# jzhou316/meta-gcn

Measured on AMD Instinct MI355X. Metric: edges/sec GCN fwd+bwd, 10M-edge synth graph F=128, at 1/2/4/8 MI355X, higher is better.
Workload: dtype f32; 1 GPU; config2: Erdos-Renyi N=1M, E=10M (+1M self-loops), F=128, 3-layer GCN (sm, add, bias, ReLU) fwd+bwd; nodes=1000000, edges=10000000, nnz=11000000, feat=128, layers=3, global_batch=1, parallelism=single

## Files before the change

meta-gcn_amd/csrc/fused.hip:

```cpp

#include <string>

#include "mgcn_internal.h"
#include "x6.h"

#ifndef MGCN_NT_AUX
#define MGCN_NT_AUX 2
#endif
#ifndef MGCN_NT_OUT
#define MGCN_NT_OUT 2
#endif

namespace mgcn {
namespace {

using namespace x6;

constexpr int kXwF = 128;
constexpr int kXwRows = 32;
constexpr int kXwWaves = 8;
constexpr int kXwThreads = 64 * kXwWaves;
constexpr int kXwImg = kXwRows * 256;
constexpr int kXwStageLd = kXwF + 8;
constexpr int kXwStage = kXwRows * kXwStageLd * 4;
// ... 1496 lines not shown
  }
  if (EPI != EPI_STORE || HCS) {
    __syncthreads();
    if constexpr (EPI != EPI_STORE) {
      if (tid < kXwF) {
        const float *red = reinterpret_cast<const float *>(lds);
        float s = 0.0f;
#pragma unroll
        for (int l = 0; l < 16; ++l) s = __fadd_rn(s, red[l * kXwF + tid]);
        a.colsum_partial[(int64_t)blockIdx.x * kXwF + tid] = s;
      }
    }
    if (HCS && tid >= kXwF && tid < 2 * kXwF) {
      const int f = tid - kXwF;
      const float *red2 = reinterpret_cast<const float *>(lds) + 16 * kXwF;
      float s = 0.0f;
#pragma unroll
      for (int l = 0; l < 16; ++l) s = __fadd_rn(s, red2[l * kXwF + f]);
      A.hcs_partial[(int64_t)blockIdx.x * kXwF + f] = s;
    }
  }
  XTAIL_EXIT(1, n_my);
}

int g_xw_ws_full = 1;
int g_xw_ws_max = 1;

int bs_grid() {
  int dev = 0, cus = 256;
  if (hipGetDevice(&dev) != hipSuccess ||
      hipDeviceGetAttribute(&cus, hipDeviceAttributeMultiprocessorCount, dev) != hipSuccess)
    cus = 256;
  return cus;
}

template <int U, int MODE, int ROLL>
int launch_bs_ur(const XbsArgs &a, int epi, int grid, hipStream_t s) {
  if (epi == EPI_RELU_DIV)
    hipLaunchKernelGGL((spmm_xw_bwd_ws_kernel<U, EPI_RELU_DIV, MODE, ROLL>), dim3(grid),
                       dim3(kBsThreads), 0, s, a);
  else if (epi == EPI_RELU)
    hipLaunchKernelGGL((spmm_xw_bwd_ws_kernel<U, EPI_RELU, MODE, ROLL>), dim3(grid),
                       dim3(kBsThreads), 0, s, a);
  else
    hipLaunchKernelGGL((spmm_xw_bwd_ws_kernel<U, EPI_STORE, MODE, ROLL>), dim3(grid),
                       dim3(kBsThreads), 0, s, a);
  return check_launch("spmm_xw_bwd_ws_kernel");
}

int g_bs_roll = 2;

template <int U, int MODE>
int launch_bs_u(const XbsArgs &a, int epi, int grid, hipStream_t s) {
  if constexpr (MODE == kBsDwsM) {
    return launch_bs_ur<U, MODE, 0>(a, epi, grid, s);
  } else {
    return g_bs_roll == 0 ? launch_bs_ur<U, MODE, 0>(a, epi, grid, s)
                          : launch_bs_ur<U, MODE, 2>(a, epi, grid, s);
  }
}

int g_bs_dbg = 0;

int g_bs_full_unroll = 5;

template <int MODE>
int launch_bs(const XbsArgs &a, int epi, int grid, hipStream_t s) {
  if constexpr (MODE == kBsDwsM) {
    return launch_bs_u<3, MODE>(a, epi, grid, s);
  } else {
    return g_bs_full_unroll == 4 ? launch_bs_u<4, MODE>(a, epi, grid, s)
         : g_bs_full_unroll == 5 ? launch_bs_u<5, MODE>(a, epi, grid, s)
                                 : launch_bs_u<6, MODE>(a, epi, grid, s);
  }
}

int bs_prepare(XbsArgs &sa) {
  sa.dbg = MGCN_EXPERIMENT ? g_bs_dbg : 0;
  sa.spin = g_spin_limit;
  sa.err = device_error_word();
  return sa.err == nullptr ? MGCN_EHIP : MGCN_OK;
}

}

int xw_set_ws(const char *name, int value) {
  const std::string n(name);
  auto flag = [&](int &g) {
    if (value < 0 || value > 1) {
      set_error("%s must be 0 or 1", name);
      return (int)MGCN_EINVAL;
    }
    g = value;
    return (int)MGCN_OK;
  };
  auto unroll = [&](int &g, std::initializer_list<int> ok) {
    for (int v : ok)
      if (v == value) {
        g = value;
        return (int)MGCN_OK;
      }
    set_error("%s: unsupported value %d", name, value);
    return (int)MGCN_EINVAL;
  };
  if (n == "xw_pk_unroll" || n == "xw_pk_bwd_unroll") {
    if (!MGCN_EXPERIMENT) {
      set_error("%s: experiment builds only (make exp -> libmgcn_exp.so)", name);
      return MGCN_EINVAL;
    }
    return n == "xw_pk_unroll" ? unroll(g_xw_pk_unroll, {3, 4, 5, 6})
                               : unroll(g_xw_pk_bwd_unroll, {2, 3, 4});
  }
  if (n == "xw_ws_max") return flag(g_xw_ws_max);
  if (n == "xw_ws_roll") return unroll(g_bs_roll, {0, 2});
  if (n == "xw_ws_full") return flag(g_xw_ws_full);
  if (n == "xw_ws_dbg") {
    if (!MGCN_EXPERIMENT) {
      set_error("xw_ws_dbg: experiment builds only (make exp -> libmgcn_exp.so)");
      return MGCN_EINVAL;
    }
    g_bs_dbg = value;
    return MGCN_OK;
  }
  return unroll(g_bs_full_unroll, {4, 5, 6});
}

int xw_set_dyn_rounds(int value) {
  if (value < 0 || value > 64) {
    set_error("xw_dyn_rounds must be in 0 .. 64 (0: no dynamic claim)");
    return MGCN_EINVAL;
  }
  g_xw_dyn_rounds = value;
  return MGCN_OK;
}

int xw_set_unroll(int value) {
  if (value != 4 && value != 5 && value != 6 && value != 8) {
    set_error("spmm_xw_unroll must be 4, 5, 6 or 8 (5 / 6: the forward only)");
    return MGCN_EINVAL;
  }
  g_xw_unroll = value;
  return MGCN_OK;
}

}

using namespace mgcn;

extern "C" int mgcn_spmm_xw_supported(int32_t F_in, int32_t F_out, int reduce) {
  return F_in == F_out && (F_in == kXwF || F_in == 256) && gemm_precision_is_x6() &&
         (reduce == MGCN_REDUCE_SUM || reduce == MGCN_REDUCE_MEAN);
}

extern "C" int mgcn_spmm_xw_bwd_full_supported(int32_t F_in, int32_t F_out) {
  return F_in == kXwF && F_out == kXwF && gemm_precision_is_x6();
}

extern "C" size_t mgcn_spmm_xw_fwd_workspace_bytes(int32_t F_in, int32_t F_out) {
  if (F_in == kXwF && F_out == kXwF) return xw_dyn_workspace_bytes();
  return F_in == 256 && F_out == 256 ? xw_wide_workspace_bytes(false) : 0;
}

namespace {
inline bool aligned16(const void *p) { return reinterpret_cast<uintptr_t>(p) % 16 == 0; }

int check_fwd_outputs(const char *who, bool wide, int32_t F_in, const float *bias,
                      const uint32_t *relu_mask, const float *Z, int64_t ldz) {
  MGCN_REQUIRE(wide || bias == nullptr || reinterpret_cast<uintptr_t>(bias) % 4 == 0,
               "%s: bias not 4-byte aligned", who);
  MGCN_REQUIRE(relu_mask == nullptr || aligned16(relu_mask), "%s: relu_mask not 16-byte aligned",
               who);
  MGCN_REQUIRE(Z == nullptr || (ldz >= F_in && ldz % 4 == 0 && aligned16(Z) &&
                                (wide || (uint64_t)kXwRows * (uint64_t)ldz * 4u < (1ull << 31))),
               "%s: Z must have 16-byte aligned rows (ldz >= F_in)", who);
  return MGCN_OK;
}

XwArgs xw_args(int64_t n_rows, const int64_t *rowptr, const int32_t *col, const float *w,
               const float *W, int64_t ldw, const float *bias, float *Y, int64_t ldy, int reduce,
               int relu, uint32_t *relu_mask, float *Z, int64_t ldz) {
  XwArgs a{};
  a.n_rows = n_rows;
  a.rowptr = rowptr;
  a.col = col;
  a.w = w;
  a.W = W;
  a.ldw = ldw;
  a.bias = bias;
  a.Y = Y;
  a.ldy = ldy;
  a.relu_mask = relu_mask;
  a.Z = Z;
  a.ldz = ldz;
  a.mean = reduce == MGCN_REDUCE_MEAN;
  a.relu = relu != 0;
// ... 7 lines not shown
int check_bwd_outputs(const char *who, bool wide, int64_t n_rows, int32_t F_in, int32_t F_out,
                      const float *W, int64_t ldw, const float *dX, int64_t lddx,
                      const uint32_t *relu_mask, const void *workspace, size_t workspace_bytes) {
  if (wide)
    MGCN_REQUIRE(W != nullptr && ldw >= F_out && lddx >= F_in && lddx % 4 == 0 && aligned16(dX) &&
                     (uint64_t)16 * (uint64_t)lddx * 4u < (1ull << 31),
                 "%s: bad W/dX (16-byte aligned dX rows)", who);
  else
    MGCN_REQUIRE(W == nullptr || (ldw % 4 == 0 && aligned16(W)),
                 "%s: W must have 16-byte aligned rows", who);
  MGCN_REQUIRE(relu_mask == nullptr || aligned16(relu_mask), "%s: relu_mask not 16-byte aligned",
               who);
  return require_workspace(who, workspace, workspace_bytes,
                           mgcn_spmm_xw_bwd_workspace_bytes(n_rows, F_in, F_out));
}

XbArgs xb_args(int64_t n_rows, const int64_t *rowptr_t, const int32_t *col_t, const float *w_t,
               const float *row_scale, const float *W, int64_t ldw, float *dX, int64_t lddx,
               const uint32_t *relu_mask, const float *row_div, void *workspace) {
  XbArgs a{};
  a.n_rows = n_rows;
  a.rowptr = rowptr_t;
  a.col = col_t;
  a.w = w_t;
  a.row_scale = row_scale;
  a.W = W;
  a.ldw = ldw;
  a.dX = dX;
  a.lddx = lddx;
  a.relu_mask = relu_mask;
  a.row_div = row_div;
  a.dw_partial = static_cast<float *>(workspace);
  a.colsum_partial = reinterpret_cast<float *>(static_cast<char *>(workspace) +
                                               align_up((size_t)xw_grid() * kXwF * kXwF * 4, 256));
  return a;
}
}

extern "C" int mgcn_spmm_xw_fwd(int64_t n_rows, int64_t n_cols, int32_t F_in, int32_t F_out,
                                const int64_t *rowptr, const int32_t *col, const float *w,
                                const float *X, int64_t ldx, const float *W, int64_t ldw,
                                const float *bias, float *Y, int64_t ldy, int reduce, int relu,
                                uint32_t *relu_mask, float *Z, int64_t ldz, void *workspace,
                                size_t workspace_bytes, void *stream) {
  clear_error();
  if (int rc = take_device_error()) return rc;
  MGCN_REQUIRE(n_rows >= 0, "mgcn_spmm_xw_fwd: negative size");
  MGCN_REQUIRE(mgcn_spmm_xw_supported(F_in, F_out, reduce),
               "mgcn_spmm_xw_fwd: unsupported F_in=%d F_out=%d reduce=%d (needs 128 x 128 or "
               "256 x 256, sum/mean, bf16x6)",
               F_in, F_out, reduce);
  MGCN_REQUIRE(relu_mask == nullptr || relu, "mgcn_spmm_xw_fwd: relu_mask needs relu");
  if (n_rows == 0) return MGCN_OK;
  MGCN_REQUIRE(rowptr && X && W && Y, "mgcn_spmm_xw_fwd: null array");
  MGCN_REQUIRE(ldx >= F_in && ldx % 4 == 0 && reinterpret_cast<uintptr_t>(X) % 16 == 0,
               "mgcn_spmm_xw_fwd: X must have 16-byte aligned rows");
  MGCN_REQUIRE(ldw >= F_out && ldy >= F_out, "mgcn_spmm_xw_fwd: leading dimension too small");
  if (F_in == 256) {
    MGCN_REQUIRE(n_cols > 0 && (uint64_t)16 * (uint64_t)(ldy > ldz ? ldy : ldz) * 4u < (1ull << 31),
                 "mgcn_spmm_xw_fwd: leading dimension too large");
    if (int rc = check_fwd_outputs("mgcn_spmm_xw_fwd", true, F_in, bias, relu_mask, Z, ldz))
      return rc;
    MGCN_REQUIRE(ldy % 4 == 0 && aligned16(Y),
                 "mgcn_spmm_xw_fwd: Y must have 16-byte aligned rows at F = 256");
    if (int rc = require_workspace("mgcn_spmm_xw_fwd", workspace, workspace_bytes,
                                   mgcn_spmm_xw_fwd_workspace_bytes(F_in, F_out)))
      return rc;
    return xw_wide_fwd(n_rows, rowptr, col, w, X, ldx, W, ldw, bias, Y, ldy,
                       reduce == MGCN_REDUCE_MEAN, relu != 0, relu_mask, Z, ldz, workspace,
                       as_stream(stream));
  }
  MGCN_REQUIRE(n_cols > 0 && (uint64_t)n_cols * (uint64_t)ldx * 4u <= 0xfffffff0ull,
               "mgcn_spmm_xw_fwd: X must hold 1 .. 4 GiB - 1 bytes (32-bit gather offsets)");
  MGCN_REQUIRE((uint64_t)kXwRows * (uint64_t)ldy * 4u < (1ull << 31),
               "mgcn_spmm_xw_fwd: ldy too large");
  if (int rc = check_fwd_outputs("mgcn_spmm_xw_fwd", false, F_in, bias, relu_mask, Z, ldz))
    return rc;
  XwArgs a = xw_args(n_rows, rowptr, col, w, W, ldw, bias, Y, ldy, reduce, relu, relu_mask, Z, ldz);
  a.X = X;
  a.ldx = ldx;
  a.n_cols = n_cols;
  hipStream_t s = as_stream(stream);
  int rc = MGCN_OK;
  if (launch_xw_dyn(a, workspace, workspace_bytes, s, &rc)) return rc;
  return g_xw_unroll == 4 ? launch_xw<4>(a, s)
       : g_xw_unroll == 5 ? launch_xw<5>(a, s)
       : g_xw_unroll == 6 ? launch_xw<6>(a, s)
                          : launch_xw<8>(a, s);
}

extern "C" size_t mgcn_spmm_xw_bwd_workspace_bytes(int64_t n_rows, int32_t F_in, int32_t F_out) {
  (void)n_rows;
  if (F_in == 256 && F_out == 256) return xw_wide_workspace_bytes(true);
  const size_t g = (size_t)xw_grid();
  return align_up(g * kXwF * kXwF * 4, 256) + align_up(g * kXwF * 4, 256);
}

namespace {
int xw_bwd_impl(int64_t n_rows, int64_t n_cols, int32_t F_in, int32_t F_out,
                const int64_t *rowptr_t, const int32_t *col_t, const float *w_t,
                const float *row_scale, const float *dY, int64_t lddy, const float *X,
                int64_t ldx, const float *W, int64_t ldw, float *dW, int64_t lddw, int accumulate,
                float *dX, int64_t lddx, const uint32_t *relu_mask, const float *row_div,
                float *colsum, const uint32_t *win_mask, const int32_t *slot_map,
                float *dy_colsum, void *workspace, size_t workspace_bytes, void *stream) {
  if (int rc = take_device_error()) return rc;
  MGCN_REQUIRE(n_rows >= 0, "mgcn_spmm_xw_bwd: negative size");
  MGCN_REQUIRE((win_mask == nullptr) == (slot_map == nullptr),
               "mgcn_spmm_xw_bwd: win_mask and slot_map go together (max adjoint)");
  MGCN_REQUIRE(mgcn_spmm_xw_supported(F_in, F_out, MGCN_REDUCE_SUM),
               "mgcn_spmm_xw_bwd: unsupported F_in=%d F_out=%d (needs 128 x 128 or 256 x 256, "
               "bf16x6)", F_in, F_out);
  const bool dx_only = X == nullptr && dW == nullptr;
  MGCN_REQUIRE(dx_only || mgcn_spmm_xw_bwd_full_supported(F_in, F_out),
               "mgcn_spmm_xw_bwd: at F=%d only the dX-only form (X = dW = NULL)", F_in);
  MGCN_REQUIRE(dx_only || (X != nullptr && dW != nullptr && lddw >= F_out),
               "mgcn_spmm_xw_bwd: bad dW (X and dW are given together, or both NULL for dX only)");
  MGCN_REQUIRE(row_div == nullptr || relu_mask != nullptr,
               "mgcn_spmm_xw_bwd: row_div needs relu_mask");
  hipStream_t s = as_stream(stream);
  if (n_rows == 0) {
    if (dy_colsum) MGCN_HIP_TRY(hipMemsetAsync(dy_colsum, 0, sizeof(float) * F_out, s));
    if (!accumulate && dW != nullptr)
      for (int32_t r = 0; r < F_in; ++r)
        MGCN_HIP_TRY(hipMemsetAsync(dW + r * lddw, 0, sizeof(float) * F_out, s));
    if (colsum && !(dx_only && accumulate))
      MGCN_HIP_TRY(hipMemsetAsync(colsum, 0, sizeof(float) * F_in, s));
    return MGCN_OK;
  }
  MGCN_REQUIRE(!dx_only || (dX != nullptr && win_mask == nullptr),
               "mgcn_spmm_xw_bwd: the dX-only form needs dX and takes no win_mask");
  const int epi = epi_of(relu_mask, row_div);
  MGCN_REQUIRE(epi == EPI_STORE || (dX != nullptr && colsum != nullptr),
               "mgcn_spmm_xw_bwd: relu_mask needs dX and colsum");
  MGCN_REQUIRE(rowptr_t && dY, "mgcn_spmm_xw_bwd: null array");
  MGCN_REQUIRE(lddy >= F_out && lddy % 4 == 0 && reinterpret_cast<uintptr_t>(dY) % 16 == 0,
               "mgcn_spmm_xw_bwd: dY must have 16-byte aligned rows");
  if (F_in == 256) {
    MGCN_REQUIRE(dX != nullptr && win_mask == nullptr, "mgcn_spmm_xw_bwd: the dX-only form needs dX");
    if (int rc = check_bwd_outputs("mgcn_spmm_xw_bwd", true, n_rows, F_in, F_out, W, ldw, dX, lddx,
                                   relu_mask, workspace, workspace_bytes))
      return rc;
    return xw_wide_bwd_dx(n_rows, rowptr_t, col_t, w_t, row_scale, dY, lddy, W, ldw, dX, lddx,
                          relu_mask, row_div, colsum, accumulate, workspace, s);
  }
  MGCN_REQUIRE(dx_only || (ldx >= F_in && ldx % 4 == 0 && reinterpret_cast<uintptr_t>(X) % 16 == 0),
               "mgcn_spmm_xw_bwd: X must have 16-byte aligned rows");
  if (dx_only) ldx = 0;
  MGCN_REQUIRE(n_cols > 0 && (uint64_t)n_cols * (uint64_t)lddy * 4u <= 0xfffffff0ull,
               "mgcn_spmm_xw_bwd: dY must hold 1 .. 4 GiB - 1 bytes (32-bit gather offsets)");
  MGCN_REQUIRE((uint64_t)kXwRows * (uint64_t)(ldx > lddx ? ldx : lddx) * 4u < (1ull << 31),
               "mgcn_spmm_xw_bwd: leading dimension too large");
  MGCN_REQUIRE(dX == nullptr || (W != nullptr && ldw >= F_out && lddx >= F_in),
               "mgcn_spmm_xw_bwd: bad W/dX");
  if (int rc = check_bwd_outputs("mgcn_spmm_xw_bwd", false, n_rows, F_in, F_out, W, ldw, dX, lddx,
                                 relu_mask, workspace, workspace_bytes))
    return rc;
  const int64_t n_chunks = (n_rows + kXwRows - 1) / kXwRows;
  int grid = xw_grid();
  if (grid > n_chunks) grid = (int)n_chunks;
  XbArgs a = xb_args(n_rows, rowptr_t, col_t, w_t, row_scale, W, ldw, dX, lddx, relu_mask, row_div,
                     workspace);
  a.dY = dY;
  a.lddy = lddy;
  a.n_cols = n_cols;
  a.X = X;
// ... 213 lines not shown
```

meta-gcn_amd/csrc/graph.hip:

```cpp

#include <hipcub/hipcub.hpp>

#include <cstring>
#include <mutex>
#include <string>

#include "mgcn_internal.h"

namespace mgcn {

static thread_local std::string g_last_error;

void set_error(const char *fmt, ...) {
  char buf[1024];
  va_list ap;
  va_start(ap, fmt);
  vsnprintf(buf, sizeof(buf), fmt, ap);
  va_end(ap);
  g_last_error = buf;
}

void clear_error() { g_last_error.clear(); }

uint32_t g_spin_limit = kSpinLimitDefault;


namespace {
std::once_flag g_dev_err_once;
volatile unsigned *g_dev_err_host = nullptr;
unsigned *g_dev_err_dev = nullptr;
hipError_t g_dev_err_status = hipSuccess;
}

unsigned *device_error_word() {
  std::call_once(g_dev_err_once, [] {
    void *p = nullptr;
    g_dev_err_status = hipHostMalloc(&p, 64, hipHostMallocMapped | hipHostMallocCoherent |
                                                 hipHostMallocPortable);
    if (g_dev_err_status != hipSuccess) return;
    std::memset(p, 0, 64);
    void *d = nullptr;
    g_dev_err_status = hipHostGetDevicePointer(&d, p, 0);
    if (g_dev_err_status != hipSuccess) return;
    g_dev_err_host = static_cast<volatile unsigned *>(p);
    g_dev_err_dev = static_cast<unsigned *>(d);
  });
  if (g_dev_err_dev == nullptr)
    set_error("device error word: %s", hipGetErrorString(g_dev_err_status));
  return g_dev_err_dev;
}

const char *device_error_what(unsigned code) {
  switch (code) {
    case kDevErrDws: return "spmm_xw_bwd_ws_kernel (128-wide adjoint)";
    case kDevErrWide: return "spmm_xw_wide_ws_kernel (256-wide layer)";
    case kDevErrPack: return "pack_rows_kernel (single-pass pack)";
    default: return "unknown kernel";
  }
}

int take_device_error() {
  if (g_dev_err_host == nullptr) return MGCN_OK;
  const unsigned code = *g_dev_err_host;
  if (code == 0) return MGCN_OK;
  *g_dev_err_host = 0u;
  set_error("device: %s stopped at a hand-off that exceeded its spin bound; "
            "the outputs of that launch are invalid (code %u)",
            device_error_what(code), code);
  return MGCN_EDEVICE;
}

namespace {

constexpr int kBlock = 256;

__global__ __launch_bounds__(kBlock) void prep_keys_kernel(
    const int64_t *__restrict__ key, const int64_t *__restrict__ other,
    int64_t nnz, int64_t n_key, int64_t n_other, int32_t *__restrict__ key32,
    int32_t *__restrict__ iota, int *__restrict__ bad) {
  int local_bad = 0;
  for (int64_t i = blockIdx.x * (int64_t)blockDim.x + threadIdx.x; i < nnz;
       i += (int64_t)gridDim.x * blockDim.x) {
    const int64_t k = key[i];
    const int64_t o = other[i];
    local_bad |= (k < 0 || k >= n_key) ? 1 : 0;
    local_bad |= (o < 0 || o >= n_other) ? 2 : 0;
    key32[i] = static_cast<int32_t>(k);
    iota[i] = static_cast<int32_t>(i);
  }
  if (__any(local_bad != 0)) {
    if ((threadIdx.x & 63) == 0) atomicOr(bad, 3);
  }
}

__global__ __launch_bounds__(kBlock) void rowptr_kernel(
    const int32_t *__restrict__ sorted_key, int64_t nnz, int64_t n,
    int64_t *__restrict__ rowptr) {
  for (int64_t r = blockIdx.x * (int64_t)blockDim.x + threadIdx.x; r <= n;
       r += (int64_t)gridDim.x * blockDim.x) {
    int64_t lo = 0, hi = nnz;
    while (lo < hi) {
      const int64_t mid = (lo + hi) >> 1;
      if ((int64_t)sorted_key[mid] < r)
        lo = mid + 1;
      else
        hi = mid;
    }
    rowptr[r] = lo;
  }
}

__global__ __launch_bounds__(kBlock) void gather_col_kernel(
    const int64_t *__restrict__ other, const int32_t *__restrict__ eid,
    int64_t nnz, int32_t *__restrict__ col) {
  for (int64_t i = blockIdx.x * (int64_t)blockDim.x + threadIdx.x; i < nnz;
       i += (int64_t)gridDim.x * blockDim.x)
    col[i] = static_cast<int32_t>(other[eid[i]]);
}

__global__ __launch_bounds__(kBlock) void degree_norm_kernel(
    int64_t n, const int64_t *__restrict__ rowptr,
    const int32_t *__restrict__ eid, const float *__restrict__ deg_in,
    const float *__restrict__ ew, int method, float *__restrict__ deg_out,
    float *__restrict__ dinv_out) {
  for (int64_t i = blockIdx.x * (int64_t)blockDim.x + threadIdx.x; i < n;
       i += (int64_t)gridDim.x * blockDim.x) {
    float d;
    if (deg_in != nullptr) {
      d = deg_in[i];
    } else if (ew != nullptr) {
      d = 0.0f;
      for (int64_t k = rowptr[i]; k < rowptr[i + 1]; ++k) d = __fadd_rn(d, ew[eid[k]]);
    } else {
      d = static_cast<float>(rowptr[i + 1] - rowptr[i]);
    }
    deg_out[i] = d;
    float v;
    if (method == MGCN_NORM_SM)
      v = __fdiv_rn(1.0f, sqrtf(d));
// ... 170 lines not shown
```

meta-gcn_amd/csrc/mgcn_internal.h:

```cpp
#pragma once

#include <hip/hip_runtime.h>

#include <atomic>
#include <cstdarg>
#include <cstdint>
#include <cstdio>

#include "mgcn.h"

namespace mgcn {

void set_error(const char *fmt, ...);
void clear_error();

inline hipStream_t as_stream(void *s) { return reinterpret_cast<hipStream_t>(s); }

#ifndef MGCN_EXPERIMENT
#define MGCN_EXPERIMENT 0
#endif
constexpr int kDbgMask = MGCN_EXPERIMENT ? ~0 : 0;
constexpr uint32_t kSpinLimitDefault = 1u << 25;
extern uint32_t g_spin_limit;

constexpr unsigned kDevErrDws = 1;
constexpr unsigned kDevErrWide = 2;
constexpr unsigned kDevErrPack = 3;
unsigned *device_error_word();
int take_device_error();

__device__ inline void report_device_error(unsigned *err, unsigned code) {
  if (err != nullptr && (threadIdx.x & 63) == 0)
    __hip_atomic_store(err, code, __ATOMIC_RELAXED, __HIP_MEMORY_SCOPE_SYSTEM);
}

inline int check_launch(const char *what) {
  hipError_t e = hipGetLastError();
  if (e != hipSuccess) {
    set_error("%s: %s", what, hipGetErrorString(e));
    return MGCN_EHIP;
  }
  return MGCN_OK;
}

#define MGCN_HIP_TRY(call)                                                    \
  do {                                                                        \
    hipError_t _e = (call);                                                   \
    if (_e != hipSuccess) {                                                   \
      ::mgcn::set_error("%s failed: %s (%s:%d)", #call, hipGetErrorString(_e), \
                        __FILE__, __LINE__);                                  \
      return MGCN_EHIP;                                                       \
    }                                                                         \
  } while (0)

#define MGCN_REQUIRE(cond, ...)       \
  do {                                \
    if (!(cond)) {                    \
      ::mgcn::set_error(__VA_ARGS__); \
      return MGCN_EINVAL;             \
    }                                 \
  } while (0)

inline int require_workspace(const char *who, const void *workspace, size_t bytes, size_t need) {
  if (workspace != nullptr && bytes >= need) return MGCN_OK;
  set_error("%s: workspace %zu < %zu", who, bytes, need);
  return MGCN_EWORKSPACE;
}

inline size_t align_up(size_t x, size_t a) { return (x + a - 1) / a * a; }

inline unsigned grid_for(int64_t work_items, int block) {
  int64_t g = (work_items + block - 1) / block;
  if (g < 1) g = 1;
  if (g > 8192) g = 8192;
  return static_cast<unsigned>(g);
}

int gemm_set_tn_variant(int value);
int gemm_set_tn_staged(int value);
int gemm_set_precision(int value);
int gemm_precision_is_x6();
int xw_set_unroll(int value);
int xw_set_dyn_rounds(int value);
int xw_set_ws(const char *name, int value);
extern int g_fused_mask;
extern int g_rl_cap;
int launch_fold(const float *partial, int64_t splits, int64_t MN, int N, float *C, int64_t ldc,
                int accumulate, hipStream_t s);
int launch_fold_split(const float *partial, int64_t splits, int64_t MN, int N, float *C,
                      int64_t ldc, int N1, float *C2, int64_t ldc2, int accumulate, hipStream_t s);
int launch_split_reduce(const float *partial, int splits, int64_t MN, int N, float *C,
                        int64_t ldc, int accumulate, hipStream_t s);
int launch_colsum_fold(const float *partial, int64_t nparts, int N, float *out, hipStream_t s);
struct SideFold {
  const float *partial;
  int64_t parts, MN;
  int N, N1, log_eb, blocks;
  float *C, *C2;
  int64_t ldc, ldc2;
};
SideFold make_side_fold(const float *partial, int64_t parts, int64_t MN, int N, float *C,
                        int64_t ldc, int N1, float *C2, int64_t ldc2);
int launch_side_fold(const SideFold &f, hipStream_t s);

__device__ inline void side_fold_block(const SideFold &f, int b, float *red) {
  const int EB = 1 << f.log_eb, T = 256 >> f.log_eb;
  const int el = threadIdx.x & (EB - 1), g = threadIdx.x >> f.log_eb;
  const int64_t e = (int64_t)b * EB + el;
  float acc = 0.0f;
  if (e < f.MN) {
// ... 62 lines not shown
```

meta-gcn_amd/csrc/spmm.hip:

```cpp

#include <hipcub/hipcub.hpp>

#include "heavy.h"
#include "mgcn_internal.h"

namespace mgcn {
namespace {

constexpr int kWaves = 4;
constexpr int kBlock = 64 * kWaves;

template <int G>
__device__ __forceinline__ int bcast_i(int v, int group_base, int k) {
  if constexpr (G == 64) {
    return __builtin_amdgcn_readlane(v, k);
  } else {
    return __shfl(v, group_base + k, 64);
  }
}
template <int G>
__device__ __forceinline__ float bcast_f(float v, int group_base, int k) {
  return __int_as_float(bcast_i<G>(__float_as_int(v), group_base, k));
}

// ... 581 lines not shown
    }
  }
  if (n_heavy > n_giant)
    return bwd ? launch_heavy_v<BWD_SUM>(a, vec, false, stream)
               : launch_heavy_v<FWD_SUM>(a, vec, false, stream);
  return MGCN_OK;
}

int heavy_rows_join(hipStream_t stream) {
  SideStream *side = nullptr;
  if (int rc = side_stream(&side)) return rc;
  MGCN_HIP_TRY(hipStreamWaitEvent(stream, side->join, 0));
  return MGCN_OK;
}

}

using namespace mgcn;

#ifdef MGCN_HEAVY_PROFILE
extern "C" int mgcn_debug_heavy_prof(unsigned long long *host) {
  MGCN_HIP_TRY(hipDeviceSynchronize());
  MGCN_HIP_TRY(hipMemcpyFromSymbol(host, HIP_SYMBOL(g_hprof), sizeof(g_hprof)));
  return MGCN_OK;
}
#endif

extern "C" int mgcn_set_option(const char *name, int value) {
  clear_error();
  MGCN_REQUIRE(name != nullptr, "mgcn_set_option: null name");
  const std::string n(name);
  if (n == "spmm_vec") {
    MGCN_REQUIRE(value == 0 || value == 1 || value == 2 || value == 4, "spmm_vec must be 0,1,2,4");
    g_force_vec = value;
    return MGCN_OK;
  }
  if (n == "spmm_unroll") {
    MGCN_REQUIRE(value == 4 || value == 6 || value == 8 || value == 16,
                 "spmm_unroll must be 4, 6, 8 or 16");
    g_unroll = value;
    g_unroll_set = true;
    return MGCN_OK;
  }
  if (n == "heavy_lds_kb") {
    MGCN_REQUIRE(value >= 16 && value <= 160, "heavy_lds_kb must be in [16, 160]");
    g_heavy_lds = value * 1024;
    return MGCN_OK;
  }
  if (n == "heavy_block") {
    MGCN_REQUIRE(value == 256 || value == 512 || value == 1024, "heavy_block must be 256, 512 or 1024");
    g_heavy_block = value;
    return MGCN_OK;
  }
  if (n == "heavy_mid_q1") {
    MGCN_REQUIRE(value == 0 || value == 1, "heavy_mid_q1 must be 0 or 1");
    g_heavy_mid_q1 = value;
    return MGCN_OK;
  }
  if (n == "heavy_mid_lds_kb") {
    MGCN_REQUIRE(value >= 16 && value <= 160, "heavy_mid_lds_kb must be in [16, 160]");
    g_heavy_mid_lds = value * 1024;
    return MGCN_OK;
  }
  if (n == "heavy_giant_thr") {
    MGCN_REQUIRE(value >= 0, "heavy_giant_thr must be >= 0");
    g_giant_thr = value;
    return MGCN_OK;
  }
  if (n == "gemm_tn_variant") {
    MGCN_REQUIRE(value >= 0 && value <= 2, "gemm_tn_variant must be 0, 1 or 2");
    return gemm_set_tn_variant(value);
  }
  if (n == "gemm_tn_staged") {
    MGCN_REQUIRE(value == 0 || value == 1, "gemm_tn_staged must be 0 or 1");
    return gemm_set_tn_staged(value);
  }
  if (n == "gemm_precision") {
    MGCN_REQUIRE(value == 0 || value == 1, "gemm_precision must be 0 (f32) or 1 (bf16x6)");
    return gemm_set_precision(value);
  }
  if (n == "spmm_xw_unroll") return xw_set_unroll(value);
  if (n == "xw_dyn_rounds") return xw_set_dyn_rounds(value);
  if (n == "xw_ws_dbg" || n == "xw_ws_full" || n == "xw_ws_max" || n == "xw_ws_full_unroll" ||
      n == "xw_ws_roll" || n == "xw_pk_unroll" || n == "xw_pk_bwd_unroll")
    return xw_set_ws(name, value);
  if (n == "wide_pair" || n == "wide_ws" || n == "wide_dbg" || n == "wide_mfma") return wide_set_option(name, value);
  if (n == "residual_blocks") {
    MGCN_REQUIRE(value >= 64 && value <= 65536, "residual_blocks must be in [64, 65536]");
    g_rl_cap = value;
    return MGCN_OK;
  }
  if (n == "residual_fused_mask") {
    MGCN_REQUIRE(value == 0 || value == 1, "residual_fused_mask must be 0 or 1");
    g_fused_mask = value;
    return MGCN_OK;
  }
  if (n == "heavy_side_fence") {
    MGCN_REQUIRE(value == 0 || value == 1, "heavy_side_fence must be 0 or 1");
    g_side_fence = value;
    return MGCN_OK;
  }
  if (n == "ws_spin_limit") {
    if (!MGCN_EXPERIMENT) {
      set_error("ws_spin_limit: experiment builds only (make exp -> libmgcn_exp.so)");
      return MGCN_EINVAL;
    }
    MGCN_REQUIRE(value >= 1, "ws_spin_limit must be >= 1");
    g_spin_limit = (uint32_t)value;
    return MGCN_OK;
  }
  if (n == "heavy_side_stream") {
    MGCN_REQUIRE(value == 0 || value == 1, "heavy_side_stream must be 0 or 1");
    g_heavy_side = value;
    return MGCN_OK;
  }
  set_error("mgcn_set_option: unknown option '%s'", name);
  return MGCN_EINVAL;
}

static int choose_vec(int32_t F, const void *p0, int64_t ld0, const void *p1, int64_t ld1) {
  int v = pick_vec(F, p0, ld0, p1, ld1);
  if (g_force_vec != 0 && g_force_vec < v) v = g_force_vec;
  return v;
}

extern "C" int mgcn_spmm_fwd(int64_t n_rows, int32_t F, const int64_t *rowptr, const int32_t *col,
                             const int32_t *eid, const float *w, const float *H, int64_t ldh,
                             float *Y, int64_t ldy, int reduce, const float *bias, int relu,
                             int32_t *argmax, uint32_t *win_mask, uint32_t *relu_mask,
                             const int32_t *order, int64_t n_heavy, int64_t n_giant,
                             void *stream) {
  clear_error();
  MGCN_REQUIRE(n_rows >= 0 && F >= 0, "mgcn_spmm_fwd: negative size");
  MGCN_REQUIRE(relu_mask == nullptr || (relu && F <= 128),
               "mgcn_spmm_fwd: relu_mask needs relu and F <= 128");
  MGCN_REQUIRE(reduce == MGCN_REDUCE_SUM || reduce == MGCN_REDUCE_MEAN || reduce == MGCN_REDUCE_MAX,
               "mgcn_spmm_fwd: bad reduce %d", reduce);
  if (n_rows == 0 || F == 0) return MGCN_OK;
  MGCN_REQUIRE(rowptr && H && Y, "mgcn_spmm_fwd: null array");
  MGCN_REQUIRE(ldh >= F && ldy >= F, "mgcn_spmm_fwd: leading dimension < F");
  MGCN_REQUIRE(reduce != MGCN_REDUCE_MAX || argmax != nullptr || win_mask != nullptr,
               "mgcn_spmm_fwd: MAX needs argmax and/or win_mask (+ eid)");
  SpmmArgs a{};
  a.n_rows = n_rows;
  a.F = F;
  a.rowptr = rowptr;
  a.col = col;
  a.eid = eid;
  a.w = w;
  a.X = H;
  a.ldx = ldh;
  a.Y = Y;
  a.ldy = ldy;
  a.bias = bias;
  a.argmax_out = argmax;
  a.win_mask_out = reduce == MGCN_REDUCE_MAX ? win_mask : nullptr;
  a.relu_mask = relu_mask;
  MGCN_REQUIRE(order == nullptr || (0 <= n_giant && n_giant <= n_heavy && n_heavy <= n_rows),
               "spmm: need 0 <= n_giant <= n_heavy <= n_rows");
  a.order = order;
  a.n_heavy = n_heavy;
  a.n_giant = n_giant;
  a.mean = reduce == MGCN_REDUCE_MEAN;
  a.relu = relu != 0;
  int vec = choose_vec(F, H, ldh, Y, ldy);
  if (reduce == MGCN_REDUCE_MAX && argmax != nullptr &&
      reinterpret_cast<uintptr_t>(argmax) % (4 * vec))
// ... 172 lines not shown
```

Measured before the change: 6.318 billion edges/s.

## Add warp-specialized forward SpMM-XW kernel with LDS ring between gather and MFMA waves

```diff
diff --git a/meta-gcn_amd/csrc/fused.hip b/meta-gcn_amd/csrc/fused.hip
--- a/meta-gcn_amd/csrc/fused.hip
+++ b/meta-gcn_amd/csrc/fused.hip
@@ -1602,6 +1602,255 @@
   return sa.err == nullptr ? MGCN_EHIP : MGCN_OK;
 }
 
+#ifndef MGCN_XF_RING
+#define MGCN_XF_RING 4
+#endif
+constexpr int kXfsRing = MGCN_XF_RING;
+constexpr int kXfsLead = 4;
+constexpr int kXfsStageOff = kXfsRing * kBsImgSet;
+constexpr int kXfsCtrOff = kXfsStageOff + 2 * kXfStage;
+constexpr int kXfsLds = kXfsCtrOff + 256;
+static_assert(kXfsRing >= 2 && kXfsRing <= 8, "ring counters: 8 words each");
+static_assert(kXfsLds <= 160 * 1024, "one forward workgroup per CU");
+
+struct XfsArgs {
+  XwArgs a;
+  uint32_t spin;
+  unsigned *err;
+};
+
+template <int U>
+__global__ __launch_bounds__(kBsThreads) void spmm_xw_fwd_ws_kernel(const XfsArgs A) {
+  const XwArgs &a = A.a;
+  __shared__ __attribute__((aligned(16))) char lds[kXfsLds];
+  const int tid = threadIdx.x;
+  const int lane = tid & 63;
+  const int wave = __builtin_amdgcn_readfirstlane(tid >> 6);
+  const int gl = lane & 31, grp = lane >> 5;
+  int *ctr = reinterpret_cast<int *>(lds + kXfsCtrOff);
+  int *filled = ctr, *mdone = ctr + 8, *freed = ctr + 16, *cid = ctr + 24, *tslot = ctr + 32;
+  int *staged = ctr + 48, *tpub = ctr + 49, *abort_word = ctr + 50;
+  if (tid < 64) ctr[tid] = 0;
+  __syncthreads();
+
+  const int64_t n_chunks = (a.n_rows + kXwRows - 1) / kXwRows;
+  const bool dyn = a.dyn_first >= 0;
+  auto rows_in = [&](int c) -> uint32_t {
+    const int64_t r = a.n_rows - (int64_t)c * kXwRows;
+    return (uint32_t)(r >= kXwRows ? kXwRows : r);
+  };
+
+  if (wave < kBsNG) {
+    const int n_stat = (int)my_chunks(dyn ? (int64_t)a.dyn_first : n_chunks);
+    auto stat_chunk = [&](int i) -> int {
+      return i < n_stat ? (int)(blockIdx.x + i * gridDim.x) : -1;
+    };
+    auto row_of = [&](int c, int second) -> int64_t {
+      return (int64_t)c * kXwRows + 4 * wave + 2 * second + grp;
+    };
+    const auto rx = buf_rsrc(a.X, (uint32_t)(a.n_cols * a.ldx * 4));
+    const uint32_t ldx_b = (uint32_t)a.ldx * 4u;
+    int c0 = stat_chunk(0), c1 = stat_chunk(1);
+    RowMeta cur[2] = {}, nxt[2] = {};
+#pragma unroll
+    for (int j = 0; j < 2; ++j) {
+      meta_rowptr(a.rowptr, row_of(c0, j), c0 >= 0 && row_of(c0, j) < a.n_rows, cur[j]);
+      meta_first(a.col, a.w, gl, cur[j]);
+      meta_rowptr(a.rowptr, row_of(c1, j), c1 >= 0 && row_of(c1, j) < a.n_rows, nxt[j]);
+    }
+    RollWin<U> win;
+    roll_first<U>(rx, ldx_b, cur[0], cur[1], gl, grp, win);
+    int k = 0, b = 0, gen = 0;
+    while (c0 >= 0) {
+      uint32_t ticket = 0;
+      const bool draw = dyn && wave == 0 && k + kXfsLead >= n_stat;
+      if (draw && lane == 0)
+        ticket = __hip_atomic_fetch_add(a.claim, 1u, __ATOMIC_RELAXED, __HIP_MEMORY_SCOPE_AGENT);
+      int c2 = stat_chunk(k + 2);
+      if (dyn && k + 2 >= n_stat) {
+        if (!bs_wait_ge(tpub, k + 3, abort_word, A.spin)) break;
+        c2 = bs_lds_load(tslot + ((k + 2) & 15));
+      }
+      RowMeta nn[2];
+#pragma unroll
+      for (int j = 0; j < 2; ++j) {
+        meta_first(a.col, a.w, gl, nxt[j]);
+        const int64_t r2 = row_of(c2, j);
+        meta_rowptr_raw(a.rowptr, r2, c2 >= 0 && r2 < a.n_rows, nn[j]);
+      }
+      const int64_t r0 = (int64_t)c0 * kXwRows;
+      const int lr0 = 4 * wave + grp;
+      float rsc[2] = {1.0f, 1.0f};
+      float acc[2][4];
+      gather_row2_roll<U>(rx, ldx_b, a.rowptr, a.col, a.w, r0 + lr0, r0 + lr0 + 2, cur[0], cur[1],
+                          nxt[0], nxt[1], c1 >= 0, gl, grp, acc[0], acc[1], win, nullptr, a.n_rows,
+                          rsc);
+      if (a.Z != nullptr) {
+        const auto rz = buf_rsrc(a.Z + r0 * a.ldz, rows_in(c0) * (uint32_t)a.ldz * 4u);
+#pragma unroll
+        for (int j = 0; j < 2; ++j)
+          __builtin_amdgcn_raw_buffer_store_b128(
+              __builtin_bit_cast(u32x4, make_float4(acc[j][0], acc[j][1], acc[j][2], acc[j][3])),
+              rz, 4 * (int)((lr0 + 2 * j) * a.ldz + 4 * gl), 0, MGCN_NT_AUX);
+      }
+      if (a.mean) {
+#pragma unroll
+        for (int j = 0; j < 2; ++j) {
+          const float c = (float)(cur[j].deg > 1 ? cur[j].deg : 1);
+#pragma unroll
+          for (int t = 0; t < 4; ++t) acc[j][t] = __fdiv_rn(acc[j][t], c);
+        }
+      }
+      if (!bs_wait_ge(freed + b, gen, abort_word, A.spin)) break;
+      char *buf = lds + b * kBsImgSet;
+#pragma unroll
+      for (int j = 0; j < 2; ++j) store_row_terms(buf, lr0 + 2 * j, gl, acc[j]);
+      if (wave == 0 && lane == 0)
+        __hip_atomic_store(cid + b, c0, __ATOMIC_RELAXED, __HIP_MEMORY_SCOPE_WORKGROUP);
+      bs_signal(filled + b, 4, lane);
+      if (draw) {
+        const uint32_t c = (uint32_t)a.dyn_first + (uint32_t)__builtin_amdgcn_readfirstlane(ticket);
+        if (lane == 0) {
+          __hip_atomic_store(tslot + ((k + kXfsLead) & 15), c < (uint32_t)n_chunks ? (int)c : -1,
+                             __ATOMIC_RELAXED, __HIP_MEMORY_SCOPE_WORKGROUP);
+          __hip_atomic_store(tpub, k + kXfsLead + 1, __ATOMIC_RELAXED,
+                             __HIP_MEMORY_SCOPE_WORKGROUP);
+        }
+      }
+#pragma unroll
+      for (int j = 0; j < 2; ++j) {
+        cur[j] = nxt[j];
+        nxt[j] = nn[j];
+        meta_deg(nxt[j]);
+      }
+      c0 = c1;
+      c1 = c2;
+      ++k;
+      if (++b == kXfsRing) {
+        b = 0;
+        ++gen;
+      }
+    }
+    if (wave == 0 && bs_wait_ge(freed + b, gen, abort_word, A.spin)) {
+      if (lane == 0)
+        __hip_atomic_store(cid + b, -1, __ATOMIC_RELAXED, __HIP_MEMORY_SCOPE_WORKGROUP);
+      bs_signal(filled + b, kXwRows, lane);
+    }
+  } else {
+    const int m = wave - kBsNG;
+    const int mt = tid - 64 * kBsNG;
+    const int l16 = lane & 15, g4 = lane >> 4;
+    const bool has_b = a.bias != nullptr;
+    const int ncol = 16 * m + l16;
+    bf16x8 wb[4][3];
+    {
+      const float *wp = a.W + (int64_t)(8 * g4) * a.ldw + ncol;
+#pragma unroll
+      for (int ks = 0; ks < 4; ++ks) {
+        float v[8];
+#pragma unroll
+        for (int j = 0; j < 8; ++j) v[j] = wp[(int64_t)(32 * ks + j) * a.ldw];
+        split3_bf16(v, wb[ks][0], wb[ks][1], wb[ks][2]);
+      }
+    }
+    const float bcol = has_b ? a.bias[ncol] : 0.0f;
+    auto flush = [&](int c, const float *stage) {
+      const int64_t r0 = (int64_t)c * kXwRows;
+      const uint32_t rin = rows_in(c);
+      const auto ry = buf_rsrc(a.Y + r0 * a.ldy, rin * (uint32_t)a.ldy * 4u);
+#pragma unroll
+      for (int h = 0; h < 2; ++h) {
+        const int lr = 16 * h + (mt >> 5);
+        const float4 v = *reinterpret_cast<const float4 *>(stage + lr * kXwF + 4 * gl);
+        __builtin_amdgcn_raw_buffer_store_b128(__builtin_bit_cast(u32x4, v), ry,
+                                               4 * (int)(lr * a.ldy + 4 * gl), 0, MGCN_NT_OUT);
+        if (a.relu_mask != nullptr) {
+          const uint32_t m0 = (uint32_t)(__ballot(v.x > 0.0f) >> (32 * grp));
+          const uint32_t m1 = (uint32_t)(__ballot(v.y > 0.0f) >> (32 * grp));
+          const uint32_t m2 = (uint32_t)(__ballot(v.z > 0.0f) >> (32 * grp));
+          const uint32_t m3 = (uint32_t)(__ballot(v.w > 0.0f) >> (32 * grp));
+          if (gl == 0 && (uint32_t)lr < rin)
+            *reinterpret_cast<uint4 *>(a.relu_mask + (r0 + lr) * 4) = make_uint4(m0, m1, m2, m3);
+        }
+      }
+    };
+    int b = 0, gen = 0, prev = -1;
+    for (int i = 0;; ++i) {
+      if (i > 0) {
+        if (!bs_wait_ge(staged, kBsNM * i, abort_word, A.spin)) break;
+        flush(prev, reinterpret_cast<const float *>(lds + kXfsStageOff + ((i - 1) & 1) * kXfStage));
+      }
+      if (!bs_wait_ge(filled + b, kXwRows * (gen + 1), abort_word, A.spin)) break;
+      const int c = bs_lds_load(cid + b);
+      if (c < 0) break;
+      const char *buf = lds + b * kBsImgSet;
+      f32x4_t acc2[2];
+#pragma unroll
+      for (int t = 0; t < 2; ++t)
+#pragma unroll
+        for (int r = 0; r < 4; ++r) acc2[t][r] = 0.0f;
+#pragma unroll
+      for (int ks = 0; ks < 4; ++ks) mfma_rows(buf, wb[ks], ks, l16, g4, acc2);
+      const int old = bs_signal(mdone + b, 1, lane);
+      if (old == kBsNM * gen + kBsNM - 1) bs_signal(freed + b, 1, lane);
+      float *stage = reinterpret_cast<float *>(lds + kXfsStageOff + (i & 1) * kXfStage);
+#pragma unroll
+      for (int t = 0; t < 2; ++t)
+#pragma unroll
+        for (int r = 0; r < 4; ++r) {
+          float v = acc2[t][r];
+          if (has_b) v = __fadd_rn(v, bcol);
+          if (a.relu) v = (v < 0.0f) ? 0.0f : v;
+          stage[(16 * t + 4 * g4 + r) * kXwF + ncol] = v;
+        }
+      bs_signal(staged, 1, lane);
+      prev = c;
+      if (++b == kXfsRing) {
+        b = 0;
+        ++gen;
+      }
+    }
+  }
+  __syncthreads();
+  if (wave == 0 && bs_lds_load(abort_word) != 0) report_device_error(A.err, kDevErrFwdWs);
+}
+
+int g_xw_fwd_ws = 1;
+
+bool launch_xw_ws(const XwArgs &a0, void *workspace, size_t workspace_bytes, hipStream_t s,
+                  int *rc) {
+  const int64_t n_chunks = (a0.n_rows + kXwRows - 1) / kXwRows;
+  if (g_xw_fwd_ws == 0 || g_xw_unroll != 5 || workspace == nullptr ||
+      reinterpret_cast<uintptr_t>(workspace) % 4 != 0 ||
+      workspace_bytes < xw_dyn_workspace_bytes() || n_chunks >= (int64_t(1) << 30))
+    return false;
+  XfsArgs A{};
+  A.a = a0;
+  A.spin = g_spin_limit;
+  A.err = device_error_word();
+  if (A.err == nullptr) {
+    *rc = MGCN_EHIP;
+    return true;
+  }
+  const int64_t grid = bs_grid();
+  const int64_t rounds = n_chunks / grid;
+  int64_t tail = 2 * (int64_t)g_xw_dyn_rounds;
+  if (tail > rounds - 8) tail = rounds - 8;
+  static_assert(kXfsLead <= 8, "static rounds before the claimed tail");
+  A.a.dyn_first = -1;
+  if (tail > 0) {
+    A.a.dyn_first = (int32_t)((rounds - tail) * grid);
+    A.a.claim = static_cast<uint32_t *>(workspace);
+    if (hipMemsetAsync(A.a.claim, 0, sizeof(uint32_t), s) != hipSuccess) {
+      *rc = check_launch("hipMemsetAsync");
+      return true;
+    }
+  }
+  hipLaunchKernelGGL((spmm_xw_fwd_ws_kernel<5>), dim3((unsigned)grid), dim3(kBsThreads), 0, s, A);
+  *rc = check_launch("spmm_xw_fwd_ws_kernel");
+  return true;
+}
+
 }
 
 int xw_set_ws(const char *name, int value) {
@@ -1631,6 +1880,7 @@
     return n == "xw_pk_unroll" ? unroll(g_xw_pk_unroll, {3, 4, 5, 6})
                                : unroll(g_xw_pk_bwd_unroll, {2, 3, 4});
   }
+  if (n == "xw_fwd_ws") return flag(g_xw_fwd_ws);
   if (n == "xw_ws_max") return flag(g_xw_ws_max);
   if (n == "xw_ws_roll") return unroll(g_bs_roll, {0, 2});
   if (n == "xw_ws_full") return flag(g_xw_ws_full);
@@ -1804,6 +2054,7 @@
   a.n_cols = n_cols;
   hipStream_t s = as_stream(stream);
   int rc = MGCN_OK;
+  if (launch_xw_ws(a, workspace, workspace_bytes, s, &rc)) return rc;
   if (launch_xw_dyn(a, workspace, workspace_bytes, s, &rc)) return rc;
   return g_xw_unroll == 4 ? launch_xw<4>(a, s)
        : g_xw_unroll == 5 ? launch_xw<5>(a, s)
diff --git a/meta-gcn_amd/csrc/graph.hip b/meta-gcn_amd/csrc/graph.hip
--- a/meta-gcn_amd/csrc/graph.hip
+++ b/meta-gcn_amd/csrc/graph.hip
@@ -55,6 +55,7 @@
     case kDevErrDws: return "spmm_xw_bwd_ws_kernel (128-wide adjoint)";
     case kDevErrWide: return "spmm_xw_wide_ws_kernel (256-wide layer)";
     case kDevErrPack: return "pack_rows_kernel (single-pass pack)";
+    case kDevErrFwdWs: return "spmm_xw_fwd_ws_kernel (128-wide forward)";
     default: return "unknown kernel";
   }
 }
diff --git a/meta-gcn_amd/csrc/mgcn_internal.h b/meta-gcn_amd/csrc/mgcn_internal.h
--- a/meta-gcn_amd/csrc/mgcn_internal.h
+++ b/meta-gcn_amd/csrc/mgcn_internal.h
@@ -26,6 +26,7 @@
 constexpr unsigned kDevErrDws = 1;
 constexpr unsigned kDevErrWide = 2;
 constexpr unsigned kDevErrPack = 3;
+constexpr unsigned kDevErrFwdWs = 4;
 unsigned *device_error_word();
 int take_device_error();
 
diff --git a/meta-gcn_amd/csrc/spmm.hip b/meta-gcn_amd/csrc/spmm.hip
--- a/meta-gcn_amd/csrc/spmm.hip
+++ b/meta-gcn_amd/csrc/spmm.hip
@@ -687,7 +687,7 @@
   if (n == "spmm_xw_unroll") return xw_set_unroll(value);
   if (n == "xw_dyn_rounds") return xw_set_dyn_rounds(value);
   if (n == "xw_ws_dbg" || n == "xw_ws_full" || n == "xw_ws_max" || n == "xw_ws_full_unroll" ||
-      n == "xw_ws_roll" || n == "xw_pk_unroll" || n == "xw_pk_bwd_unroll")
+      n == "xw_ws_roll" || n == "xw_fwd_ws" || n == "xw_pk_unroll" || n == "xw_pk_bwd_unroll")
     return xw_set_ws(name, value);
   if (n == "wide_pair" || n == "wide_ws" || n == "wide_dbg" || n == "wide_mfma") return wide_set_option(name, value);
   if (n == "residual_blocks") {
```

After: 6.416 billion edges/s, median of 6. 1.02x the previous value.
